# t0saki/YOLO-Infer-pt

Hardware: AMD Instinct MI355X
Metric: images/sec at 640x640 batch32, v11_n (forward + on-device NMS) (higher is better)
Workload: dtype bf16; 1 GPU; yolo_v11_n eval forward + NMS, 640x640, 32 images per GPU per step; per_gpu_batch=32, global_batch=32, image_size=640, parallelism=dp1, nms=on-device, conf 0.001, iou 0.65, max_det 300

## Files before the change

### yolo-infer-pt_amd/csrc/c3k2.hip

```cpp
#include "common.h"
#include "dtypes.h"

namespace yh {

namespace {

typedef float f32x16 __attribute__((ext_vector_type(16)));

template <typename T> struct CMfma;
template <> struct CMfma<__bf16> {
    static __device__ __forceinline__ f32x16 step(const uint4& a, const uint4& b, const f32x16& c) {
        return __builtin_amdgcn_mfma_f32_32x32x16_bf16(__builtin_bit_cast(bf16x8, a), __builtin_bit_cast(bf16x8, b), c, 0,
                                                       0, 0);
    }
};
template <> struct CMfma<_Float16> {
    static __device__ __forceinline__ f32x16 step(const uint4& a, const uint4& b, const f32x16& c) {
        return __builtin_amdgcn_mfma_f32_32x32x16_f16(__builtin_bit_cast(f16x8, a), __builtin_bit_cast(f16x8, b), c, 0, 0,
                                                      0);
    }
};

constexpr int NWV = CSP_THREADS / 64;

__device__ __forceinline__ void cs_glds(const void* src, unsigned lds_addr) {
#if defined(__HIP_DEVICE_COMPILE__)
    unsigned keep;
    asm volatile("s_mov_b32 %0, m0\n\ts_mov_b32 m0, %2\n\ts_nop 0\n\tglobal_load_lds_dwordx4 %1, off\n\ts_mov_b32 m0, %0"
                 : "=&s"(keep) : "v"(src), "s"(lds_addr) : "memory");
#else
    (void)src; (void)lds_addr;
#endif
}
__device__ __forceinline__ void cs_barrier() { asm volatile("s_waitcnt lgkmcnt(0)\n\ts_barrier" ::: "memory"); }

__device__ __forceinline__ uint4 cs_rd(unsigned addr) {
#if defined(__HIP_DEVICE_COMPILE__)
    typedef __attribute__((address_space(3))) const uint4* lp;
    return *reinterpret_cast<lp>((size_t)addr);
#else
    (void)addr;
    return uint4{};
#endif
}
__device__ __forceinline__ void cs_wr(unsigned addr, uint4 v) {
#if defined(__HIP_DEVICE_COMPILE__)
    typedef __attribute__((address_space(3))) uint4* lp;
    *reinterpret_cast<lp>((size_t)addr) = v;
#else
    (void)addr; (void)v;
#endif
}
__device__ __forceinline__ float4 cs_rdf(unsigned addr) {
    const uint4 u = cs_rd(addr);
    return make_float4(__uint_as_float(u.x), __uint_as_float(u.y), __uint_as_float(u.z), __uint_as_float(u.w));
}

struct CsLayout {
    int w1, w2, w3, w4, b1, b2, b3, b4, prm;
};
__host__ __device__ constexpr CsLayout cs_layout(int ni, int nc, int no) {
    const int nh = (nc + 1) / 2, na3 = (nc + 1) / 2;
    CsLayout L{};
    L.w1 = 0;
    L.w2 = L.w1 + nc * ni * 1024;
    L.w3 = L.w2 + 9 * nc * 1024;
    L.w4 = L.w3 + na3 * 9 * nh * 1024;
    L.b1 = L.w4 + no * 3 * nc * 1024;
    L.b2 = L.b1 + 32 * nc * 4;
    L.b3 = L.b2 + 32 * 4;
    L.b4 = L.b3 + 32 * na3 * 4;
    L.prm = (L.b4 + 32 * no * 4 + 1023) & ~1023;
    return L;
}
struct CsTile {
    int lx, lt, lr, lc, total;
};
__host__ __device__ inline CsTile cs_tile(int TH, int TW, int ni, int nc, int no) {
    const int nh = (nc + 1) / 2;
    const CsLayout L = cs_layout(ni, nc, no);
    const int XP = (TH + 4) * (TW + 4), MP = (TH + 2) * (TW + 2), NP = TH * TW;
    CsTile t{};
    t.lx = L.prm;
    t.lt = t.lx + (ni ? ((XP * (16 * ni + 8) * 2 + 1023) & ~1023) : 0);
    t.lr = t.lt + XP * (32 * nc + 8) * 2;
    t.lc = t.lr + MP * (16 * nh + 8) * 2;
    t.total = t.lc + NP * (16 * nc + 8) * 2;
    return t;
}

template <typename T>
__device__ __forceinline__ void cs_act(const f32x16& acc, unsigned bias_addr, uint4 (&o)[2]) {
    float v[16];
#pragma unroll
    for (int q = 0; q < 4; ++q) {
        const float4 b = cs_rdf(bias_addr + 16 * q);
        v[4 * q] = acc[4 * q] + b.x;
        v[4 * q + 1] = acc[4 * q + 1] + b.y;
        v[4 * q + 2] = acc[4 * q + 2] + b.z;
        v[4 * q + 3] = acc[4 * q + 3] + b.w;
    }
    T t[16];
#pragma unroll
    for (int i = 0; i < 16; ++i) t[i] = fromf<T>(silu<T>(v[i]));
    o[0] = *reinterpret_cast<const uint4*>(&t[0]);
    o[1] = *reinterpret_cast<const uint4*>(&t[8]);
}

template <typename T, int NA, int NK, typename BAddr, typename Epi>
__device__ __forceinline__ void cs_phase(unsigned aimg, int npx, BAddr baddr, Epi epi) {
    const int lane = threadIdx.x & 63, wv = threadIdx.x >> 6, l32 = lane & 31;
    const int items = NA * ((npx + 31) >> 5);
    for (int i0 = wv; i0 < items; i0 += 2 * NWV) {
        const int i1 = i0 + NWV;
        const int a0 = i0 % NA, a1 = i1 % NA;
        const int p0 = (i0 / NA) * 32 + l32, p1 = (i1 / NA) * 32 + l32;
        const int c0 = p0 < npx ? p0 : npx - 1, c1 = p1 < npx ? p1 : npx - 1;
        const unsigned ai0 = aimg + (unsigned)(a0 * NK * 1024 + lane * 16);
        const unsigned ai1 = aimg + (unsigned)(a1 * NK * 1024 + lane * 16);
        f32x16 acc0, acc1;
#pragma unroll
        for (int e = 0; e < 16; ++e) { acc0[e] = 0.f; acc1[e] = 0.f; }
        if (i1 < items) {
#pragma unroll
            for (int k = 0; k < NK; ++k) {
                const uint4 f0 = cs_rd(ai0 + k * 1024), f1 = NA > 1 ? cs_rd(ai1 + k * 1024) : f0;
                const uint4 x0 = cs_rd(baddr(c0, k)), x1 = cs_rd(baddr(c1, k));
                acc0 = CMfma<T>::step(f0, x0, acc0);
                acc1 = CMfma<T>::step(f1, x1, acc1);
            }
            if (p0 < npx) epi(a0, p0, acc0);
            if (p1 < npx) epi(a1, p1, acc1);
        } else {
#pragma unroll
            for (int k = 0; k < NK; ++k) acc0 = CMfma<T>::step(cs_rd(ai0 + k * 1024), cs_rd(baddr(c0, k)), acc0);
            if (p0 < npx) epi(a0, p0, acc0);
        }
    }
}

template <typename T, int NI, int NC, int NO>
__global__ __launch_bounds__(CSP_THREADS) void csp_fused(const CspArgs A) {
    constexpr int NH = (NC + 1) / 2, NA3 = (NC + 1) / 2;
    constexpr int SX = 16 * NI + 8, ST = 32 * NC + 8, SR = 16 * NH + 8, SC = 16 * NC + 8;
    constexpr CsLayout L = cs_layout(NI, NC, NO);
    extern __shared__ __attribute__((aligned(16))) char sm[];
    typedef __attribute__((address_space(3))) char* lds_c;
    const unsigned lds0 = (unsigned)(size_t)(lds_c)sm;
    const int TH = A.TH, TW = A.TW, XW = TW + 4, MW = TW + 2;
    const int XP = (TH + 4) * XW, MP = (TH + 2) * MW, NP = TH * TW;
    const CsTile G = cs_tile(TH, TW, NI, NC, NO);
    const unsigned LX = lds0 + G.lx, LT = lds0 + G.lt, LR = lds0 + G.lr, LC = lds0 + G.lc;
    const int lane = threadIdx.x & 63, hh = lane >> 5;
    const int wvu = __builtin_amdgcn_readfirstlane(threadIdx.x >> 6);
    const T* x = reinterpret_cast<const T*>(A.x);
    T* y = reinterpret_cast<T*>(A.y);

    {
        const char* prm = reinterpret_cast<const char*>(A.prm);
        for (int i0 = wvu * 64; i0 < L.prm / 16; i0 += CSP_THREADS) cs_glds(prm + (size_t)(i0 + lane) * 16, lds0 + i0 * 16);
    }
    constexpr bool TAIL = NI == 0;
    constexpr int NCH = TAIL ? 4 * NC : 2 * NI;
    constexpr int CPX = NCH + 1;
    const unsigned LD = TAIL ? LT : LX;
    auto load_x = [&](int t) {
        const int n = t / A.tiles, tix = t - n * A.tiles;
        const int ty = tix / A.ntw, tx = tix - ty * A.ntw;
        const int h0 = ty * TH - 2, w0 = tx * TW - 2;
        const int total = XP * CPX;
        for (int i0 = wvu * 64; i0 < total; i0 += CSP_THREADS) {
            const int q = i0 + lane;
            const int px = q / CPX, c = q - px * CPX;
            const int r = px / XW, cc = px - r * XW;
            const int gh = h0 + r, gw = w0 + cc;
            const bool ok = q < total && c < NCH && (unsigned)gh < (unsigned)A.H && (unsigned)gw < (unsigned)A.W;
            const void* src = ok ? (const void*)(x + (((long long)n * A.H + gh) * A.W + gw) * A.ldx + c * 8) : A.zero;
            cs_glds(src, LD + i0 * 16);
        }
    };
    const int t0 = xcd_remap(blockIdx.x, gridDim.x);
    if (t0 < A.ntiles) load_x(t0);

    for (int t = t0; t < A.ntiles; t += gridDim.x) {
        const int n = t / A.tiles, tix = t - n * A.tiles;
        const int ty = tix / A.ntw, tx = tix - ty * A.ntw;
        const int h0 = ty * TH, w0 = tx * TW;
        asm volatile("s_waitcnt vmcnt(0)" ::: "memory");
        cs_barrier();

        if constexpr (!TAIL) {
        cs_phase<T, NC, NI>(
                lds0 + L.w1, XP,
                [&](int px, int k) { return LX + (unsigned)(px * SX + 16 * k + 8 * hh) * 2; },
                [&](int a, int px, const f32x16& acc) {
                    uint4 o[2];
                    cs_act<T>(acc, lds0 + L.b1 + (32 * a + 16 * hh) * 4, o);
                    const int r = px / XW, cc = px - r * XW;
                    const int gh = h0 - 2 + r, gw = w0 - 2 + cc;
                    if (!((unsigned)gh < (unsigned)A.H && (unsigned)gw < (unsigned)A.W)) o[0] = o[1] = make_uint4(0, 0, 0, 0);
                    const unsigned d = LT + (unsigned)(px * ST + 32 * a + 16 * hh) * 2;
                    cs_wr(d, o[0]);
                    cs_wr(d + 16, o[1]);
                });
        cs_barrier();
        if (t + (int)gridDim.x < A.ntiles) load_x(t + gridDim.x);
        }

        cs_phase<T, 1, 9 * NC>(
            lds0 + L.w2, MP,
            [&](int px, int k) {
                const int cb = k / 9, tap = k - 9 * (k / 9), kh = tap / 3, kw = tap - 3 * (tap / 3);
                const int r = px / MW, cc = px - r * MW;
                return LT + (unsigned)(((r + kh) * XW + cc + kw) * ST + 16 * NC + 16 * cb + 8 * hh) * 2;
            },
            [&](int, int px, const f32x16& acc) {
                if (16 * hh >= 16 * NH) return;
                uint4 o[2];
                cs_act<T>(acc, lds0 + L.b2 + 16 * hh * 4, o);
                const int r = px / MW, cc = px - r * MW;
                const int gh = h0 - 1 + r, gw = w0 - 1 + cc;
                if (!((unsigned)gh < (unsigned)A.H && (unsigned)gw < (unsigned)A.W)) o[0] = o[1] = make_uint4(0, 0, 0, 0);
                const unsigned d = LR + (unsigned)(px * SR + 16 * hh) * 2;
                cs_wr(d, o[0]);
                cs_wr(d + 16, o[1]);
            });
        cs_barrier();

        cs_phase<T, NA3, 9 * NH>(
                lds0 + L.w3, NP,
                [&](int px, int k) {
                    const int cb = k / 9, tap = k - 9 * (k / 9), kh = tap / 3, kw = tap - 3 * (tap / 3);
                    const int r = px / TW, cc = px - r * TW;
                    return LR + (unsigned)(((r + kh) * MW + cc + kw) * SR + 16 * cb + 8 * hh) * 2;
                },
                [&](int a, int px, const f32x16& acc) {
                    const int co = 32 * a + 16 * hh;
                    if (co >= 16 * NC) return;
                    uint4 o[2];
                    cs_act<T>(acc, lds0 + L.b3 + co * 4, o);
                    const int r = px / TW, cc = px - r * TW;
                    const unsigned rs = LT + (unsigned)(((r + 2) * XW + cc + 2) * ST + 16 * NC + co) * 2;
#pragma unroll
                    for (int hf = 0; hf < 2; ++hf) {
                        const uint4 rv = cs_rd(rs + 16 * hf);
                        const T* ov = reinterpret_cast<const T*>(&o[hf]);
                        const T* rr = reinterpret_cast<const T*>(&rv);
                        T s[8];
#pragma unroll
                        for (int e = 0; e < 8; ++e) s[e] = fromf<T>(tof(ov[e]) + tof(rr[e]));
                        o[hf] = *reinterpret_cast<const uint4*>(s);
                    }
                    const unsigned d = LC + (unsigned)(px * SC + co) * 2;
                    cs_wr(d, o[0]);
                    cs_wr(d + 16, o[1]);
                });
        cs_barrier();

        cs_phase<T, NO, 3 * NC>(
                lds0 + L.w4, NP,
                [&](int px, int k) {
                    const int r = px / TW, cc = px - r * TW;
                    return k < 2 * NC ? LT + (unsigned)(((r + 2) * XW + cc + 2) * ST + 16 * k + 8 * hh) * 2
                                      : LC + (unsigned)(px * SC + 16 * (k - 2 * NC) + 8 * hh) * 2;
                },
                [&](int a, int px, const f32x16& acc) {
                    uint4 o[2];
                    const int co = 32 * a + 16 * hh;
                    cs_act<T>(acc, lds0 + L.b4 + co * 4, o);
                    const int r = px / TW, cc = px - r * TW;
                    const int gh = h0 + r, gw = w0 + cc;
                    if ((unsigned)gh < (unsigned)A.H && (unsigned)gw < (unsigned)A.W) {
                        uint4* d = reinterpret_cast<uint4*>(y + (((long long)n * A.H + gh) * A.W + gw) * A.ldy + co);
                        d[0] = o[0];
                        d[1] = o[1];
                    }
                });
        if constexpr (TAIL) {
            cs_barrier();
            if (t + (int)gridDim.x < A.ntiles) load_x(t + gridDim.x);
        }
    }
    asm volatile("s_waitcnt vmcnt(0)" ::: "memory");
}

#define YH_CSP_LIST(X) X(2, 1, 2) X(4, 2, 4) X(0, 2, 2) X(0, 2, 4)

template <typename T>
int launch_csp_t(const CspArgs& a, int grid, hipStream_t s) {
    const int lds = csp_lds(a.TH, a.TW, a.ni, a.nc, a.no);
    if (lds == 0 || grid <= 0 || a.ldx % 8 || a.ldy % 8) return (int)hipErrorInvalidValue;
#define YH_CSP_CASE(NI, NC, NO)                                                                              \
    if (a.ni == NI && a.nc == NC && a.no == NO) {                                                            \
        static bool attr = false;                                                                            \
        if (!attr) {                                                                                         \
            (void)hipFuncSetAttribute(reinterpret_cast<const void*>(&csp_fused<T, NI, NC, NO>),              \
                                      hipFuncAttributeMaxDynamicSharedMemorySize, 160 * 1024);               \
            attr = true;                                                                                     \
        }                                                                                                    \
        hipLaunchKernelGGL((csp_fused<T, NI, NC, NO>), dim3((unsigned)grid), dim3(CSP_THREADS), lds, s, a); \
        return (int)hipGetLastError();                                                                       \
    }
    YH_CSP_LIST(YH_CSP_CASE)
#undef YH_CSP_CASE
    return (int)hipErrorInvalidValue;
}

}

int csp_prm_bytes(int ni, int nc, int no) { return cs_layout(ni, nc, no).prm; }

void csp_offsets(int ni, int nc, int no, int (&off)[9]) {
    const CsLayout L = cs_layout(ni, nc, no);
    const int v[9] = {L.w1, L.w2, L.w3, L.w4, L.b1, L.b2, L.b3, L.b4, L.prm};
    for (int i = 0; i < 9; ++i) off[i] = v[i];
}

int csp_lds(int TH, int TW, int ni, int nc, int no) {
    bool inst = false;
#define YH_CSP_HAS(NI, NC, NO) inst = inst || (ni == NI && nc == NC && no == NO);
    YH_CSP_LIST(YH_CSP_HAS)
#undef YH_CSP_HAS
    if (!inst || TH < 1 || TW < 1) return 0;
    const int b = cs_tile(TH, TW, ni, nc, no).total;
    return b <= 160 * 1024 ? b : 0;
}

int launch_csp(int dtype, const CspArgs& a, int grid, hipStream_t s) {
    switch (dtype) {
        case F16: return launch_csp_t<_Float16>(a, grid, s);
        case BF16: return launch_csp_t<__bf16>(a, grid, s);
    }
    return (int)hipErrorInvalidValue;
}

}
```

### yolo-infer-pt_amd/csrc/engine.cpp

```cpp
#include <hip/hip_runtime.h>

#include <algorithm>
#include <cmath>
#include <cstdio>
#include <cstring>
#include <map>
#include <memory>
#include <stdexcept>
#include <string>
#include <vector>

#include "common.h"
#include "conv_mx.h"
#include "match_host.h"
#include "merge_host.h"
#include "yolo_hip.h"


namespace yh {

static thread_local std::string g_err;

struct Fail : std::runtime_error {
    int code;
// ... 92 lines not shown
    std::vector<Seg> in;
    View out, res;
    bool has_res = false;
    int heads = 0;
    View lvl[3];
    int hc[3][5] = {};
    View hx[3], hy[3];
    bool hlv[3] = {false, false, false};
    bool direct = false;
    int bc[3] = {-1, -1, -1};
    View bx[3];
    int dlo = 0;
    bool dbox = true;
    int cs[4] = {-1, -1, -1, -1};
    int ck[7] = {-1, -1, -1, -1, -1, -1, -1};
    int alt0 = -1, alt1 = -1;
    int bxc[3][3] = {{-1, -1, -1}, {-1, -1, -1}, {-1, -1, -1}};
    std::vector<int> alts;
    struct PwRun { int stage = -1; int coff = 0; int nch = 0; int load = -1; };
    struct PwStage { std::vector<PwRun> runs; int res_stage = -2; int res_coff = 0; int res_load = -1; bool keep = false; int lds = -1; };
    std::vector<PwStage> pws;
    std::vector<View> pwl;
    std::vector<int> pwl_lds;
    int pwP = 0, pwLds = 0;
    std::string label;
};

struct Workspace {
    int B = 0, H = 0, W = 0;
    void* base = nullptr;
    size_t bytes = 0;
    std::vector<size_t> off;
};

struct GraphKey {
    int B, H, W;
    int X = 0;
    bool operator<(const GraphKey& o) const {
        return B != o.B ? B < o.B : (H != o.H ? H < o.H : (W != o.W ? W < o.W : X < o.X));
    }
};

struct Options {
    bool fuse = true, csp_tail = false, tune_log = false, c3k = true, hcls_wide = true, box_chain = false, pw_chain = true;
    int conv_force = -1;
    static Options from_env() {
        Options o;
        if (const char* e = getenv("YH_FUSE")) o.fuse = atoi(e) != 0;
        if (const char* e = getenv("YH_BOXCHAIN")) o.box_chain = atoi(e) != 0;
        if (const char* e = getenv("YH_PWCHAIN")) o.pw_chain = atoi(e) != 0;
        if (const char* e = getenv("YH_CSP_TAIL")) o.csp_tail = atoi(e) != 0;
        if (const char* e = getenv("YH_C3K")) o.c3k = atoi(e) != 0;
        if (const char* e = getenv("YH_HCLS_WIDE")) o.hcls_wide = atoi(e) != 0;
        if (const char* e = getenv("YH_CONV")) o.conv_force = atoi(e);
        o.tune_log = getenv("YH_TUNE_LOG") != nullptr;
        return o;
    }
};

struct Net {
    yh_variant var;
    Options opt;
    int device, dtype, es;
    std::vector<Tensor> tensors;
    std::vector<ConvDesc> convs;
    std::vector<Op> ops;
    Workspace ws;
    void** io_dev = nullptr;
    void* zero_dev = nullptr;
    bool use_graph = true;
    std::map<GraphKey, hipGraphExec_t> graphs;
    hipStream_t cap_stream = nullptr;
    bool profile = false;
    std::vector<double> prof_ms;
    std::vector<int> prof_calls;
    GraphKey prof_key{0, 0, 0};
    std::vector<hipEvent_t> ev;
    int lastB = 0, lastH = 0, lastW = 0;
    struct MxChoice { MxPlan plan; const char* w = nullptr; std::string name; };
    std::map<GraphKey, std::vector<MxChoice>> conv_kern;
    const std::vector<MxChoice>* cur_kern = nullptr;
    int force_kern = -1;
    int num_cus = 0;
    struct Unit { int first, last; bool level; };
    struct Plan {
        std::vector<Unit> units;
        std::vector<char> active;
    };
    std::map<GraphKey, Plan> plans;
    const Plan* cur_plan = nullptr;

    int tensor(int level, int C) {
        tensors.push_back({level, round_up(C, 8)});
        return (int)tensors.size() - 1;
    }
    View full(int t, int C = -1) {
        View v;
        v.t = t;
        v.coff = 0;
        v.C = C < 0 ? tensors[t].C : C;
        return v;
    }
    View slice(int t, int coff, int C) {
        require(coff % 8 == 0 && C % 8 == 0, "concat slice not a multiple of 8 channels");
        View v;
        v.t = t;
        v.coff = coff;
        v.C = C;
        return v;
    }
    int new_conv(const std::string& name, ConvKind kind, int cin, int cout, int k, int s, int g, int has_bias, int act) {
        ConvDesc d;
        d.name = name;
        d.kind = kind;
        d.cin = cin; d.cout = cout; d.k = k; d.stride = s; d.groups = g;
        d.has_bias = has_bias; d.act = act;
        convs.push_back(std::move(d));
        return (int)convs.size() - 1;
    }
    void dense(const std::string& name, const std::vector<Seg>& in, const std::vector<int>& logical, int cout, int k,
               int s, int act, View out, const View* res = nullptr, int has_bias = 0) {
        int cin = 0;
        for (int c : logical) cin += c;
        const int ci = new_conv(name, CK_DENSE, cin, cout, k, s, 1, has_bias, act);
        ConvDesc& d = convs[ci];
        for (size_t i = 0; i < in.size(); ++i) d.segs.push_back({logical[i], in[i].v.C});
        require(in.size() <= 2, "at most two concat segments");
        if (in.size() == 2) require(logical[0] == in[0].v.C && logical[0] % 8 == 0, "segment 0 must be 8-aligned");
        Op op;
        op.kind = OP_CONV;
        op.conv = ci;
        op.in = in;
        op.out = out;
        if (res) { op.res = *res; op.has_res = true; }
        op.label = name;
        ops.push_back(op);
    }
    View conv1(const std::string& name, View x, int xc, int cout, int act, View out, const View* res = nullptr) {
        dense(name, {Seg{x, 0}}, {xc}, cout, 1, 1, act, out, res);
        return out;
    }
    View conv3(const std::string& name, View x, int xc, int cout, int s, int act, View out, const View* res = nullptr) {
        dense(name, {Seg{x, 0}}, {xc}, cout, 3, s, act, out, res);
        return out;
    }

    void residual(const std::string& p, View x, int ch, double e, View out, int level) {
        const int hid = (int)(ch * e);
        const int t = tensor(level, hid);
        conv3(p + ".conv1", x, ch, hid, 1, ACT_SILU, full(t));
        conv3(p + ".conv2", full(t), hid, ch, 1, ACT_SILU, out, &x);
    }
    void cspmodule(const std::string& p, View x, int in_ch, int out_ch, View out, int level) {
        const int h = out_ch / 2;
        const int t = tensor(level, 2 * h);
        View a = slice(t, 0, h), b = slice(t, h, h);
        const int a0 = tensor(level, h), a1 = tensor(level, h);
        const int first = (int)ops.size();
        conv1(p + ".conv1", x, in_ch, h, ACT_SILU, full(a0));
        conv1(p + ".conv2", x, in_ch, h, ACT_SILU, b);
        residual(p + ".res_m.0", full(a0), h, 1.0, full(a1), level);
        residual(p + ".res_m.1", full(a1), h, 1.0, a, level);
        conv1(p + ".conv3", full(t), 2 * h, out_ch, ACT_SILU, out);
        if (dtype != F32 && opt.fuse && opt.c3k && (in_ch == 64 || in_ch == 128) && out_ch == in_ch && x.C == in_ch &&
            x.coff % 8 == 0 && out.coff % 8 == 0) {
            Op op;
// ... 333 lines not shown
                }
            }
        }
        if ((int)ch.pwl.size() > PWC_MAX_LOADS) return false;
        auto layout = [&](int P) {
            int off = 0;
            for (int k = 0; k < n; ++k) {
                Op::PwStage& st = ch.pws[k];
                st.lds = -1;
                if (!st.keep) continue;
                st.lds = off;
                off += (P * (convs[ops[i + k].conv].cout + 8) * 2 + 15) & ~15;
            }
            ch.pwl_lds.assign(ch.pwl.size(), 0);
            for (size_t z = 0; z < ch.pwl.size(); ++z) {
                off = (off + 1023) & ~1023;
                ch.pwl_lds[z] = off;
                off += (P * (ch.pwl[z].C + 8) * 2 + 1023) & ~1023;
            }
            off = (off + 1023) & ~1023;
            return off + 1024;
        };
        int P = 64, lds = layout(64);
        if (lds > 160 * 1024) {
            P = 32;
            lds = layout(32);
        }
        if (lds > 160 * 1024) return false;
        ch.pwP = P;
        ch.pwLds = lds;
        for (int k = 0; k < n; ++k) ch.alts.push_back((int)(i + k));
        ch.label = ops[i].label + " +" + std::to_string(n - 1);
        ch.out = ops[e - 1].out;
        for (auto& o : ops) {
            if (o.alt0 >= (int)e) o.alt0++;
            if (o.alt1 >= (int)e) o.alt1++;
            for (int& k : o.alts)
                if (k >= (int)e) k++;
        }
        ops.insert(ops.begin() + e, ch);
        return true;
    }
    int new_dense_conv(const std::string& name, int cin, int cout, int k, int has_bias, int act) {
        const int ci = new_conv(name, CK_DENSE, cin, cout, k, 1, 1, has_bias, act);
        convs[ci].segs.push_back({cin, round_up(cin, 8)});
        return ci;
    }
    bool fuse_stem(int c0, int c1, int c2) const {
        if (dtype == F32 || !opt.fuse) return false;
        return c0 == 3 && stem2_ok(c1, c2);
    }
    const void* stem2_params(const Op& op, int& bias_off) {
        ConvDesc& d = convs[op.cs[0]];
        const int nt = d.cout / 32, nk = 9 * (d.cin / 16);
        bias_off = nt * nk * 1024;
        auto it = d.mx_w.find("stem2");
        if (it != d.mx_w.end()) return it->second;
        require(d.loaded, "weights of " + d.name + " not loaded", YH_ESTATE);
        std::vector<uint8_t> img((size_t)bias_off + (size_t)d.cout * 4, 0);
        uint16_t* dst = reinterpret_cast<uint16_t*>(img.data());
        for (int a = 0; a < nt; ++a)
            for (int k = 0; k < nk; ++k)
                for (int lane = 0; lane < 64; ++lane)
                    for (int j = 0; j < 8; ++j) {
                        const int R = lane & 31, hh = lane >> 5;
                        const int co = 32 * a + 16 * ((R >> 2) & 1) + (R & 3) + 4 * (R >> 3);
                        const int cb = k / 9, tap = k - cb * 9, ch = 16 * cb + 8 * hh + j;
                        const float v = d.wf[((size_t)co * d.cin + ch) * 9 + tap];
                        dst[((size_t)(a * nk + k) * 64 + lane) * 8 + j] = dtype == BF16 ? f2bf(v) : f2h(v);
                    }
        float* bd = reinterpret_cast<float*>(img.data() + bias_off);
        for (int i = 0; i < d.cout; ++i) bd[i] = d.bf[i];
        void* dev = nullptr;
        HIPCHECK(hipMalloc(&dev, img.size()));
        HIPCHECK(hipMemcpy(dev, img.data(), img.size(), hipMemcpyHostToDevice));
        d.mx_w.emplace("stem2", dev);
        return dev;
    }
    bool fuse_csp(const std::vector<Seg>& in, const std::vector<int>& logical, int c, int out_ch, View out) const {
        if (dtype == F32 || !opt.fuse) return false;
        if (in.size() != 1 || in[0].up || in[0].v.C != logical[0] || logical[0] % 16 || c % 16 || out_ch % 32) return false;
        if (out.coff % 8 || in[0].v.coff % 8) return false;
        int TH, TW;
        return csp_tile(logical[0] / 16, c / 16, out_ch / 32, 1 << 30, 1 << 30, TH, TW);
    }
    bool fuse_csp_tail(int c, int out_ch, View out) const {
        if (dtype == F32 || !opt.fuse) return false;
        if (c % 16 || out_ch % 32 || out.coff % 8) return false;
        int TH, TW;
        return csp_tile(0, c / 16, out_ch / 32, 1 << 30, 1 << 30, TH, TW);
    }
    bool tail_first() const { return opt.csp_tail; }
    static bool csp_tile(int ni, int nc, int no, int H, int W, int& TH, int& TW) {
        if (const char* e = getenv("YH_CSP_TILE")) {
            int th = 0, tw = 0;
            if (sscanf(e, "%dx%d", &th, &tw) == 2 && th > 0 && tw > 0 && th <= H && tw <= W &&
                csp_lds(th, tw, ni, nc, no) > 0) {
                TH = th;
                TW = tw;
                return true;
            }
        }
        static const int cand[][2] = {{8, 32}, {16, 16}, {8, 16}, {8, 8}, {4, 16}, {4, 8}, {2, 8}, {2, 4}};
        const bool wide = CSP_THREADS >= 1024;
        for (int lim : {80 * 1024, 160 * 1024})
            for (auto& c : cand) {
                if (wide && lim == 80 * 1024) break;
                if (!wide && c[0] * c[1] > 128) continue;
                if (c[0] > H || c[1] > W || (lim == 80 * 1024 && c[0] * c[1] < 64)) continue;
                const int b = csp_lds(c[0], c[1], ni, nc, no);
                if (b > 0 && b <= lim) {
                    TH = c[0];
                    TW = c[1];
                    return true;
                }
            }
        return false;
    }
    const void* csp_params(const Op& op) {
        const int k0 = op.cs[0] >= 0 ? 0 : 1;
        ConvDesc& d0 = convs[op.cs[k0]];
        auto it = d0.mx_w.find("csp");
        bool ok = it != d0.mx_w.end();
        for (int k = k0 + 1; k < 4; ++k) ok = ok && convs[op.cs[k]].mx_w.count("csp_dep");
        if (ok) return it->second;
        if (it != d0.mx_w.end()) {
            (void)hipFree(it->second);
            d0.mx_w.erase(it);
        }
        for (int k = k0; k < 4; ++k) require(convs[op.cs[k]].loaded, "weights of " + convs[op.cs[k]].name + " not loaded", YH_ESTATE);
        const ConvDesc &r1 = convs[op.cs[1]], &r2 = convs[op.cs[2]], &c2 = convs[op.cs[3]];
        const int ni = k0 == 0 ? convs[op.cs[0]].cin / 16 : 0, nc = r1.cin / 16, no = c2.cout / 32, nh = (nc + 1) / 2;
        int off[9];
        csp_offsets(ni, nc, no, off);
        std::vector<uint8_t> img((size_t)off[8], 0);
        auto frags = [&](int o, const ConvDesc& d, int ntile, int nk) {
            const int kk2 = d.k * d.k;
            uint16_t* dst = reinterpret_cast<uint16_t*>(img.data() + o);
            for (int a = 0; a < ntile; ++a)
                for (int k = 0; k < nk; ++k)
                    for (int lane = 0; lane < 64; ++lane)
                        for (int j = 0; j < 8; ++j) {
                            const int R = lane & 31, hh = lane >> 5;
                            const int co = 32 * a + 16 * ((R >> 2) & 1) + (R & 3) + 4 * (R >> 3);
                            const int cb = k / kk2, tap = k - cb * kk2, ch = 16 * cb + 8 * hh + j;
                            float v = 0.f;
                            if (co < d.cout && ch < d.cin) v = d.wf[((size_t)co * d.cin + ch) * kk2 + tap];
                            dst[((size_t)(a * nk + k) * 64 + lane) * 8 + j] = dtype == BF16 ? f2bf(v) : f2h(v);
                        }
        };
        if (ni) frags(off[0], convs[op.cs[0]], nc, ni);
        frags(off[1], r1, 1, 9 * nc);
        frags(off[2], r2, nh, 9 * nh);
        frags(off[3], c2, no, 3 * nc);
        auto biases = [&](int o, const ConvDesc& d) {
            float* dst = reinterpret_cast<float*>(img.data() + o);
            for (int i = 0; i < d.cout; ++i) dst[i] = d.bf[i];
        };
        if (ni) biases(off[4], convs[op.cs[0]]);
        biases(off[5], r1);
        biases(off[6], r2);
        biases(off[7], c2);
        void* dev = nullptr;
        HIPCHECK(hipMalloc(&dev, img.size()));
        HIPCHECK(hipMemcpy(dev, img.data(), img.size(), hipMemcpyHostToDevice));
        d0.mx_w.emplace("csp", dev);
        for (int k = k0 + 1; k < 4; ++k) convs[op.cs[k]].mx_w.emplace("csp_dep", nullptr);
        return dev;
    }
    const void* c3k_params(const Op& op) {
        ConvDesc& d0 = convs[op.ck[0]];
        auto it = d0.mx_w.find("c3k");
        bool ok = it != d0.mx_w.end();
        for (int k = 1; k < 7; ++k) ok = ok && convs[op.ck[k]].mx_w.count("c3k_dep");
        if (ok) return it->second;
        if (it != d0.mx_w.end()) {
            (void)hipFree(it->second);
            d0.mx_w.erase(it);
        }
        for (int k = 0; k < 7; ++k) require(convs[op.ck[k]].loaded, "weights of " + convs[op.ck[k]].name + " not loaded", YH_ESTATE);
        const int hh = convs[op.ck[0]].cout, nt3 = hh / 32, nk1 = hh / 8, nk3 = 9 * hh / 16;
        int off[9];
        c3k_offsets(hh, off);
        std::vector<uint8_t> img((size_t)off[8], 0);
        auto frags = [&](int o, const ConvDesc& d, int ntile, int nk, bool rho) {
            const int kk2 = d.k * d.k;
            uint16_t* dst = reinterpret_cast<uint16_t*>(img.data() + o);
            for (int a = 0; a < ntile; ++a)
                for (int k = 0; k < nk; ++k)
                    for (int lane = 0; lane < 64; ++lane)
                        for (int j = 0; j < 8; ++j) {
// ... 698 lines not shown
                a.H = H; a.W = W; a.Ho = H >> 1; a.Wo = W >> 1;
                a.Cout = d.cout_p;
                a.ldo = ldc(op.out);
                a.M = B * a.Ho * a.Wo;
                a.w = (const float*)d.w_dev;
                a.bias = d.b_dev;
                a.out = ptr(op.out);
                a.act = d.act;
                a.in_u8 = in_u8;
                rc = launch_first_conv(dtype, a, B, s);
                break;
            }
            case OP_CONV: {
                if (dtype != F32) {
                    require(cur_kern != nullptr, "conv plans not chosen", YH_ESTATE);
                    rc = launch_mx_op(op, (*cur_kern)[oi].plan, B, H, W, s);
                    break;
                }
                ConvArgs a{};
                int BM, BN;
                conv_args(op, B, H, W, a, BM, BN);
                rc = launch_conv(dtype, CONV_GEMM, BM, BN, a, s);
                break;
            }
            case OP_DW: rc = launch_dwconv(dtype, dw_args(op, B, H, W), s); break;
            case OP_SPPF: rc = launch_sppf(dtype, pool_args(op, B, H, W), s); break;
            case OP_ATTN: rc = launch_attention(dtype, attn_args(op, H, W), B, s); break;
            case OP_HEADCLS: {
                rc = launch_head_cls(dtype, head_cls_args(op, B, H, W), s);
                break;
            }
            case OP_DECODE: {
                DecodeArgs a{};
                for (int l = 0; l < 3; ++l) {
                    const Tensor& t = tensors[op.lvl[l].t];
                    a.lvl[l] = ptr(op.lvl[l]);
                    a.H[l] = H >> t.level; a.W[l] = W >> t.level;
                    a.stride[l] = (float)(1 << t.level);
                    a.ldc = t.C;
                }
                a.nc = var.num_classes;
                a.A = a.H[0] * a.W[0] + a.H[1] * a.W[1] + a.H[2] * a.W[2];
                a.B = B;
                a.io = (const void* const*)io_dev;
                a.a_lo = anchor_off(op.dlo, H, W);
                a.box = op.dbox ? 1 : 0;
                rc = launch_decode(dtype, a, s);
                break;
            }
            case OP_BOXDFL: rc = launch_box_dfl(dtype, box_dfl_args(op, B, H, W), s); break;
            case OP_BOXCHAIN: rc = launch_box_chain(dtype, box_chain_args(op, B, H, W), s); break;
            case OP_PWCHAIN: rc = launch_pw_chain(dtype, pw_chain_args(op, B, H, W), op.pwLds, s); break;
            case OP_STEM2: {
                const ConvDesc& d = convs[op.conv];
                Stem2Args a{};
                a.io = (const void* const*)io_dev;
                a.H = H; a.W = W; a.Hs = H >> 1; a.Ws = W >> 1; a.Ho = H >> 2; a.Wo = W >> 2; a.B = B;
                a.w1 = (const float*)d.w_dev;
                a.b1 = d.b_dev;
                a.c1 = d.cout; a.c1p = d.cout_p; a.c2 = convs[op.cs[0]].cout;
                a.prm = stem2_params(op, a.prm_bias);
                a.out = ptr(op.out);
                a.ldo = ldc(op.out);
                a.in_u8 = in_u8;
                stem2_tiles(a.Ho, a.Wo, a.ntw, a.nth);
                rc = launch_stem2(dtype, a, s);
                break;
            }
            case OP_CSP: {
                CspArgs a{};
                const View& xv = op.in[0].v;
                const int lv = tensors[xv.t].level;
                a.x = ptr(xv);
                a.ldx = ldc(xv);
                a.y = ptr(op.out);
                a.ldy = ldc(op.out);
                a.H = H >> lv;
                a.W = W >> lv;
                a.B = B;
                a.prm = csp_params(op);
                a.ni = op.cs[0] >= 0 ? convs[op.cs[0]].cin / 16 : 0;
                a.nc = convs[op.cs[1]].cin / 16;
                a.no = convs[op.cs[3]].cout / 32;
                require(csp_tile(a.ni, a.nc, a.no, a.H, a.W, a.TH, a.TW), op.label + ": no LDS tile");
                a.ntw = (a.W + a.TW - 1) / a.TW;
                a.tiles = a.ntw * ((a.H + a.TH - 1) / a.TH);
                a.ntiles = B * a.tiles;
                a.zero = zero_dev;
                if (!num_cus) HIPCHECK(hipDeviceGetAttribute(&num_cus, hipDeviceAttributeMultiprocessorCount, device));
                {
                    const int lds = csp_lds(a.TH, a.TW, a.ni, a.nc, a.no);
                    const int per_cu = CSP_THREADS < 1024 && lds > 0 && lds <= 80 * 1024 ? 2 : 1;
                    rc = launch_csp(dtype, a, std::min(a.ntiles, per_cu * num_cus), s);
                }
                break;
            }
            case OP_C3K: {
                C3kArgs a{};
                const View& xv = op.in[0].v;
                const int lv = tensors[xv.t].level;
                a.x = ptr(xv);
                a.ldx = ldc(xv);
                a.y = ptr(op.out);
                a.ldy = ldc(op.out);
                a.H = H >> lv;
                a.W = W >> lv;
                a.B = B;
                a.prm = c3k_params(op);
                a.hh = convs[op.ck[0]].cout;
                rc = launch_c3k(dtype, a, s);
                break;
            }
        }
        if (rc != 0) throw Fail(YH_EHIP, "launch of " + op.label + " failed: " + hipGetErrorString((hipError_t)rc));
    }

    void free_plans() {
        plans.clear();
        cur_plan = nullptr;
    }
    void ensure_plan(int B, int H, int W) {
        const GraphKey key{B, H, W};
        auto it = plans.find(key);
        if (it != plans.end()) { cur_plan = &it->second; return; }
        Plan pl;
        pl.active.assign(ops.size(), 1);
        for (size_t i = 0; i < ops.size(); ++i) {
            if (ops[i].kind != OP_BOXCHAIN) continue;
            bool fits = true;
            for (int l = 0; l < 3; ++l) {
                const int lv = tensors[ops[i].hx[l].t].level;
                int th, tw;
                fits = fits && bx_tile(H >> lv, W >> lv, th, tw);
            }
            if (fits)
                for (int k : ops[i].alts) pl.active[k] = 0;
            else
                pl.active[i] = 0;
        }
        for (size_t i = 0; i < ops.size(); ++i) {
            if (ops[i].kind != OP_PWCHAIN) continue;
            const int lv = tensors[ops[i].out.t].level;
            const long long M = (long long)B * (H >> lv) * (W >> lv);
            const double grid = (double)((M + ops[i].pwP - 1) / ops[i].pwP);
            double wb = 0;
            for (int k : ops[i].alts) wb += (double)convs[ops[k].conv].cout * convs[ops[k].conv].K * es;
            if (wb * grid <= 160e6)
                for (int k : ops[i].alts) pl.active[k] = 0;
            else
                pl.active[i] = 0;
        }
        for (size_t i = 0; i < ops.size(); ++i) {
            if (ops[i].kind != OP_C3K) continue;
            const int lv = tensors[ops[i].out.t].level;
            if (c3k_lds(H >> lv, W >> lv, convs[ops[i].ck[0]].cout) > 0)
                for (int k = ops[i].alt0; k < ops[i].alt1; ++k) pl.active[k] = 0;
            else
                pl.active[i] = 0;
        }
        for (size_t i = 0; i < ops.size(); ++i)
            if (pl.active[i]) pl.units.push_back(Unit{(int)i, (int)i + 1, false});
        cur_plan = &plans.emplace(key, std::move(pl)).first->second;
    }
    void launch_unit(const Unit& u, int B, int H, int W, hipStream_t s) {
        for (int k = u.first; k < u.last; ++k) launch_op(k, B, H, W, s);
    }

    void run_ops(int B, int H, int W, hipStream_t s) {
        if (!cur_plan) {
            for (size_t i = 0; i < ops.size(); ++i) launch_op(i, B, H, W, s);
            return;
        }
// ... 696 lines not shown
        auto it = n.plans.find(yh::GraphKey{batch, height, width});
        yh::require(it != n.plans.end(), "no forward has run at this shape yet", YH_ESTATE);
        const auto& us = it->second.units;
        yh::require(index >= 0 && index < (int)us.size(), "unit index out of range");
        const bool prof_here = n.prof_key.B == batch && n.prof_key.H == height && n.prof_key.W == width;
        if (first_op) *first_op = us[index].first;
        if (num_ops) *num_ops = us[index].last - us[index].first;
        if (is_level) *is_level = us[index].level ? 1 : 0;
        if (ms_total) *ms_total = prof_here && index < (int)n.prof_ms.size() ? n.prof_ms[index] : 0.0;
        if (calls) *calls = prof_here && index < (int)n.prof_calls.size() ? n.prof_calls[index] : 0;
    });
}

int yh_set_graph(yh_handle* h, int enable) {
    return guarded([&] {
        yh::require(h, "null handle");
        h->net.use_graph = enable != 0;
    });
}

int yh_profile_enable(yh_handle* h, int enable) {
    return guarded([&] {
        yh::require(h, "null handle");
        h->net.profile = enable != 0;
    });
}

int yh_profile_reset(yh_handle* h) {
    return guarded([&] {
        yh::require(h, "null handle");
        std::fill(h->net.prof_ms.begin(), h->net.prof_ms.end(), 0.0);
        std::fill(h->net.prof_calls.begin(), h->net.prof_calls.end(), 0);
    });
}

int yh_force_conv_kernel(yh_handle* h, int kernel) {
    return guarded([&] {
        yh::require(h, "null handle");
        yh::require(kernel >= -1, "conv plan index out of range");
        h->net.force_kern = kernel;
        h->net.conv_kern.clear();
        h->net.cur_kern = nullptr;
        h->net.drop_graphs();
    });
}

int yh_debug_op_desc(const yh_handle* h, int index, int batch, int height, int width, char* buf, size_t size) {
    int len = 0;
    const int rc = guarded([&] {
        yh::require(h && index >= 0 && index < (int)h->net.ops.size(), "op index out of range");
        const std::string s = h->net.op_desc(index, batch, height, width);
        yh::require(buf && size > s.size(), "buffer too small");
        std::memcpy(buf, s.c_str(), s.size() + 1);
        len = (int)s.size();
    });
    return rc == YH_OK ? len : rc;
}

int yh_debug_run_ops(yh_handle* h, const void* x, int x_u8, int batch, int height, int width, void* y, int first,
                     int last, void* stream) {
    return guarded([&] {
        yh::require(h && x && y, "null argument");
        h->net.debug_run(x, x_u8, batch, height, width, y, first, last, (hipStream_t)stream);
    });
}

int yh_debug_operand(const yh_handle* h, int index, int slot, void* dst, size_t dst_bytes, void* stream) {
    return guarded([&] {
        yh::require(h && dst, "null argument");
        HIPCHECK(hipSetDevice(h->net.device));
        h->net.debug_operand(index, slot, dst, dst_bytes, (hipStream_t)stream);
    });
}

int yh_op_count(const yh_handle* h) { return h ? (int)h->net.ops.size() : YH_EINVAL; }

int yh_op_kernel(const yh_handle* h, int index, int batch, int height, int width, const char** name) {
    return guarded([&] {
        yh::require(h && index >= 0 && index < (int)h->net.ops.size(), "op index out of range");
        const yh::Net& n = h->net;
        const yh::Op& op = n.ops[index];
        if (op.kind != yh::OP_CONV) {
            if (name) *name = yh::op_kind_name(op.kind);
            return;
        }
        if (n.dtype == yh::F32) {
            if (name) *name = "gemm_f32";
            return;
        }
        auto it = n.conv_kern.find(yh::GraphKey{batch, height, width});
        yh::require(it != n.conv_kern.end(), "no forward has run at this shape yet", YH_ESTATE);
        if (name) *name = it->second[index].name.c_str();
    });
}

int yh_op_info(const yh_handle* h, int index, int batch, int height, int width, const char** label, int* op_class,
               double* bytes, double* flops, double* ms_total, int* calls) {
    return guarded([&] {
        yh::require(h && index >= 0 && index < (int)h->net.ops.size(), "op index out of range");
        const yh::Net& n = h->net;
        const yh::Op& op = n.ops[index];
        if (label) *label = op.label.c_str();
        if (op_class) *op_class = (int)n.op_class(op);
        double b = 0, f = 0;
        n.op_cost(op, batch, height, width, b, f);
        if (bytes) *bytes = b;
        if (flops) *flops = f;
        double ms = 0.0;
        int nc = 0;
        auto it = n.plans.find(yh::GraphKey{batch, height, width});
        const bool prof_here = n.prof_key.B == batch && n.prof_key.H == height && n.prof_key.W == width;
        if (it != n.plans.end() && prof_here) {
            const auto& us = it->second.units;
            for (size_t u = 0; u < us.size() && u < n.prof_ms.size(); ++u)
                if (!us[u].level && us[u].first == index) { ms = n.prof_ms[u]; nc = n.prof_calls[u]; }
        }
        if (ms_total) *ms_total = ms;
        if (calls) *calls = nc;
    });
}

}
```

Measured before the change: 40700 images/s.

## Cost-model CSP tile selection, relax store wait, and half-width epilogues for single-block stages

Replaces the fixed candidate list for the fused C3k2 tile with a cost model that weighs per-tile fixed overhead against MFMA item count and the number of tile waves over CUs. It also replaces the full vmcnt(0) wait at the top of each tile with a partial wait that lets the previous tile's output stores stay in flight. It adds permlane32-swap based half-width epilogues when the hidden or channel block count is one, so both lane halves do useful work instead of idling. Optional trace instrumentation is compiled out by default. The risks are a poorly calibrated cost model picking bad tiles and subtle correctness problems in the partial wait counting.

```diff
diff --git a/yolo-infer-pt_amd/csrc/c3k2.hip b/yolo-infer-pt_amd/csrc/c3k2.hip
--- a/yolo-infer-pt_amd/csrc/c3k2.hip
+++ b/yolo-infer-pt_amd/csrc/c3k2.hip
@@ -33,6 +33,21 @@
 #endif
 }
 __device__ __forceinline__ void cs_barrier() { asm volatile("s_waitcnt lgkmcnt(0)\n\ts_barrier" ::: "memory"); }
+
+__device__ __forceinline__ void cs_wait_vm(int n) {
+    if (n >= 8) asm volatile("s_waitcnt vmcnt(8)" ::: "memory");
+    else if (n >= 4) asm volatile("s_waitcnt vmcnt(4)" ::: "memory");
+    else if (n >= 2) asm volatile("s_waitcnt vmcnt(2)" ::: "memory");
+    else asm volatile("s_waitcnt vmcnt(0)" ::: "memory");
+}
+
+#ifdef YH_CSP_TRACE
+constexpr int CS_TR = 12, CS_TR_TILES = 16, CS_TR_WG = 256, CS_TR_OPS = 4;
+__device__ unsigned long long csp_trace_buf[CS_TR_OPS * CS_TR_WG * CS_TR_TILES * CS_TR];
+#define CS_STAMP(k) do { if (trp) trp[k] = __builtin_amdgcn_s_memtime(); } while (0)
+#else
+#define CS_STAMP(k) do { } while (0)
+#endif
 
 __device__ __forceinline__ uint4 cs_rd(unsigned addr) {
 #if defined(__HIP_DEVICE_COMPILE__)
@@ -107,6 +122,31 @@
     o[1] = *reinterpret_cast<const uint4*>(&t[8]);
 }
 
+template <typename T>
+__device__ __forceinline__ uint4 cs_act_half(const f32x16& acc, unsigned bias_addr, int hh) {
+#if defined(__HIP_DEVICE_COMPILE__)
+    float v[8];
+#pragma unroll
+    for (int e = 0; e < 8; ++e)
+        v[e] = __uint_as_float(
+            __builtin_amdgcn_permlane32_swap(__float_as_uint(acc[e]), __float_as_uint(acc[8 + e]), false, false)[0]);
+    const float4 b0 = cs_rdf(bias_addr + 32 * hh), b1 = cs_rdf(bias_addr + 32 * hh + 16);
+    v[0] += b0.x; v[1] += b0.y; v[2] += b0.z; v[3] += b0.w;
+    v[4] += b1.x; v[5] += b1.y; v[6] += b1.z; v[7] += b1.w;
+    T t[8];
+#pragma unroll
+    for (int i = 0; i < 8; ++i) {
+        float p = silu<T>(v[i]);
+        asm("" : "+v"(p));
+        t[i] = fromf<T>(p);
+    }
+    return *reinterpret_cast<const uint4*>(&t[0]);
+#else
+    (void)acc; (void)bias_addr; (void)hh;
+    return uint4{};
+#endif
+}
+
 template <typename T, int NA, int NK, typename BAddr, typename Epi>
 __device__ __forceinline__ void cs_phase(unsigned aimg, int npx, BAddr baddr, Epi epi) {
     const int lane = threadIdx.x & 63, wv = threadIdx.x >> 6, l32 = lane & 31;
@@ -138,6 +178,10 @@
         }
     }
 }
+
+#ifdef YH_CSP_TRACE
+constexpr int cs_trace_op(int ni, int, int no) { return ni == 2 ? 0 : ni == 4 ? 1 : no == 2 ? 2 : 3; }
+#endif
 
 template <typename T, int NI, int NC, int NO>
 __global__ __launch_bounds__(CSP_THREADS) void csp_fused(const CspArgs A) {
@@ -182,12 +226,30 @@
     const int t0 = xcd_remap(blockIdx.x, gridDim.x);
     if (t0 < A.ntiles) load_x(t0);
 
+    const int p4_items = NO * ((NP + 31) >> 5);
+    const int p4_stores = wvu < p4_items ? 2 * ((p4_items - wvu + NWV - 1) / NWV) : 0;
+    int young = 0;
+#ifdef YH_CSP_TRACE
+    int trk = 0;
+#endif
     for (int t = t0; t < A.ntiles; t += gridDim.x) {
         const int n = t / A.tiles, tix = t - n * A.tiles;
         const int ty = tix / A.ntw, tx = tix - ty * A.ntw;
         const int h0 = ty * TH, w0 = tx * TW;
-        asm volatile("s_waitcnt vmcnt(0)" ::: "memory");
+#ifdef YH_CSP_TRACE
+        unsigned long long* trp = nullptr;
+        if (threadIdx.x == 0 && blockIdx.x < CS_TR_WG && trk < CS_TR_TILES) {
+            trp = csp_trace_buf + ((size_t)(cs_trace_op(NI, NC, NO) * CS_TR_WG + blockIdx.x) * CS_TR_TILES + trk) * CS_TR;
+            trp[10] = __builtin_amdgcn_s_memrealtime();
+            trp[11] = (unsigned long long)TH | (unsigned long long)TW << 16 | (unsigned long long)(t + 1) << 32;
+        }
+        ++trk;
+#endif
+        CS_STAMP(0);
+        cs_wait_vm(young);
+        CS_STAMP(1);
         cs_barrier();
+        CS_STAMP(2);
 
         if constexpr (!TAIL) {
         cs_phase<T, NC, NI>(
@@ -203,7 +265,9 @@
                     cs_wr(d, o[0]);
                     cs_wr(d + 16, o[1]);
                 });
+        CS_STAMP(3);
         cs_barrier();
+        CS_STAMP(4);
         if (t + (int)gridDim.x < A.ntiles) load_x(t + gridDim.x);
         }
 
@@ -215,6 +279,14 @@
                 return LT + (unsigned)(((r + kh) * XW + cc + kw) * ST + 16 * NC + 16 * cb + 8 * hh) * 2;
             },
             [&](int, int px, const f32x16& acc) {
+                if constexpr (NH == 1) {
+                    uint4 o = cs_act_half<T>(acc, lds0 + L.b2, hh);
+                    const int r = px / MW, cc = px - r * MW;
+                    const int gh = h0 - 1 + r, gw = w0 - 1 + cc;
+                    if (!((unsigned)gh < (unsigned)A.H && (unsigned)gw < (unsigned)A.W)) o = make_uint4(0, 0, 0, 0);
+                    cs_wr(LR + (unsigned)(px * SR + 8 * hh) * 2, o);
+                    return;
+                }
                 if (16 * hh >= 16 * NH) return;
                 uint4 o[2];
                 cs_act<T>(acc, lds0 + L.b2 + 16 * hh * 4, o);
@@ -225,7 +297,9 @@
                 cs_wr(d, o[0]);
                 cs_wr(d + 16, o[1]);
             });
+        CS_STAMP(5);
         cs_barrier();
+        CS_STAMP(6);
 
         cs_phase<T, NA3, 9 * NH>(
                 lds0 + L.w3, NP,
@@ -235,6 +309,18 @@
                     return LR + (unsigned)(((r + kh) * MW + cc + kw) * SR + 16 * cb + 8 * hh) * 2;
                 },
                 [&](int a, int px, const f32x16& acc) {
+                    if constexpr (NC == 1) {
+                        const uint4 o = cs_act_half<T>(acc, lds0 + L.b3, hh);
+                        const int r = px / TW, cc = px - r * TW;
+                        const uint4 rv = cs_rd(LT + (unsigned)(((r + 2) * XW + cc + 2) * ST + 16 * NC + 8 * hh) * 2);
+                        const T* ov = reinterpret_cast<const T*>(&o);
+                        const T* rr = reinterpret_cast<const T*>(&rv);
+                        T s[8];
+#pragma unroll
+                        for (int e = 0; e < 8; ++e) s[e] = fromf<T>(tof(ov[e]) + tof(rr[e]));
+                        cs_wr(LC + (unsigned)(px * SC + 8 * hh) * 2, *reinterpret_cast<const uint4*>(s));
+                        return;
+                    }
                     const int co = 32 * a + 16 * hh;
                     if (co >= 16 * NC) return;
                     uint4 o[2];
@@ -255,7 +341,9 @@
                     cs_wr(d, o[0]);
                     cs_wr(d + 16, o[1]);
                 });
+        CS_STAMP(7);
         cs_barrier();
+        CS_STAMP(8);
 
         cs_phase<T, NO, 3 * NC>(
                 lds0 + L.w4, NP,
@@ -276,6 +364,8 @@
                         d[1] = o[1];
                     }
                 });
+        CS_STAMP(9);
+        if constexpr (!TAIL) young = h0 + TH <= A.H && w0 + TW <= A.W ? p4_stores : 0;
         if constexpr (TAIL) {
             cs_barrier();
             if (t + (int)gridDim.x < A.ntiles) load_x(t + gridDim.x);
@@ -326,6 +416,13 @@
     return b <= 160 * 1024 ? b : 0;
 }
 
+#ifdef YH_CSP_TRACE
+extern "C" int yh_debug_csp_trace(unsigned long long* dst, int n) {
+    if (n > CS_TR_OPS * CS_TR_WG * CS_TR_TILES * CS_TR) n = CS_TR_OPS * CS_TR_WG * CS_TR_TILES * CS_TR;
+    return (int)hipMemcpyFromSymbol(dst, HIP_SYMBOL(csp_trace_buf), (size_t)n * 8, 0, hipMemcpyDeviceToHost);
+}
+#endif
+
 int launch_csp(int dtype, const CspArgs& a, int grid, hipStream_t s) {
     switch (dtype) {
         case F16: return launch_csp_t<_Float16>(a, grid, s);
diff --git a/yolo-infer-pt_amd/csrc/engine.cpp b/yolo-infer-pt_amd/csrc/engine.cpp
--- a/yolo-infer-pt_amd/csrc/engine.cpp
+++ b/yolo-infer-pt_amd/csrc/engine.cpp
@@ -198,6 +198,7 @@
     const std::vector<MxChoice>* cur_kern = nullptr;
     int force_kern = -1;
     int num_cus = 0;
+    std::map<std::pair<GraphKey, int>, std::string> csp_plan;
     struct Unit { int first, last; bool level; };
     struct Plan {
         std::vector<Unit> units;
@@ -697,16 +698,20 @@
         if (in.size() != 1 || in[0].up || in[0].v.C != logical[0] || logical[0] % 16 || c % 16 || out_ch % 32) return false;
         if (out.coff % 8 || in[0].v.coff % 8) return false;
         int TH, TW;
-        return csp_tile(logical[0] / 16, c / 16, out_ch / 32, 1 << 30, 1 << 30, TH, TW);
+        return csp_tile(logical[0] / 16, c / 16, out_ch / 32, 1, 1 << 30, 1 << 30, 1, TH, TW);
     }
     bool fuse_csp_tail(int c, int out_ch, View out) const {
         if (dtype == F32 || !opt.fuse) return false;
         if (c % 16 || out_ch % 32 || out.coff % 8) return false;
         int TH, TW;
-        return csp_tile(0, c / 16, out_ch / 32, 1 << 30, 1 << 30, TH, TW);
+        return csp_tile(0, c / 16, out_ch / 32, 1, 1 << 30, 1 << 30, 1, TH, TW);
     }
     bool tail_first() const { return opt.csp_tail; }
-    static bool csp_tile(int ni, int nc, int no, int H, int W, int& TH, int& TW) {
+    static int csp_items(int TH, int TW, int ni, int nc, int no) {
+        const auto nb = [](int px) { return (px + 31) / 32; };
+        return (ni ? nc * nb((TH + 4) * (TW + 4)) : 0) + nb((TH + 2) * (TW + 2)) + ((nc + 1) / 2 + no) * nb(TH * TW);
+    }
+    static bool csp_tile(int ni, int nc, int no, int B, int H, int W, int cus, int& TH, int& TW) {
         if (const char* e = getenv("YH_CSP_TILE")) {
             int th = 0, tw = 0;
             if (sscanf(e, "%dx%d", &th, &tw) == 2 && th > 0 && tw > 0 && th <= H && tw <= W &&
@@ -716,12 +721,30 @@
                 return true;
             }
         }
-        static const int cand[][2] = {{8, 32}, {16, 16}, {8, 16}, {8, 8}, {4, 16}, {4, 8}, {2, 8}, {2, 4}};
-        const bool wide = CSP_THREADS >= 1024;
+        if (CSP_THREADS >= 1024) {
+            constexpr long long CSP_TILE_FIXED = 7400, CSP_TILE_ITEM = 230;
+            long long best = -1;
+            H = std::min(H, 1 << 12);
+            W = std::min(W, 1 << 12);
+            for (int th : {2, 4, 8, 10, 12, 16}) {
+                if (th > H || (th == 2 && H >= 4)) continue;
+                for (int tw = 4; tw <= W; tw += 4) {
+                    if (csp_lds(th, tw, ni, nc, no) <= 0) break;
+                    const long long nt = (long long)B * ((H + th - 1) / th) * ((W + tw - 1) / tw);
+                    const long long cost = ((nt + cus - 1) / cus) * (CSP_TILE_FIXED + CSP_TILE_ITEM * csp_items(th, tw, ni, nc, no));
+                    if (best < 0 || cost < best) {
+                        best = cost;
+                        TH = th;
+                        TW = tw;
+                    }
+                    if (nt <= cus) break;
+                }
+            }
+            return best >= 0;
+        }
+        static const int cand[][2] = {{8, 16}, {8, 8}, {4, 16}, {4, 8}, {2, 8}, {2, 4}};
         for (int lim : {80 * 1024, 160 * 1024})
             for (auto& c : cand) {
-                if (wide && lim == 80 * 1024) break;
-                if (!wide && c[0] * c[1] > 128) continue;
                 if (c[0] > H || c[1] > W || (lim == 80 * 1024 && c[0] * c[1] < 64)) continue;
                 const int b = csp_lds(c[0], c[1], ni, nc, no);
                 if (b > 0 && b <= lim) {
@@ -1586,12 +1609,13 @@
                 a.ni = op.cs[0] >= 0 ? convs[op.cs[0]].cin / 16 : 0;
                 a.nc = convs[op.cs[1]].cin / 16;
                 a.no = convs[op.cs[3]].cout / 32;
-                require(csp_tile(a.ni, a.nc, a.no, a.H, a.W, a.TH, a.TW), op.label + ": no LDS tile");
+                if (!num_cus) HIPCHECK(hipDeviceGetAttribute(&num_cus, hipDeviceAttributeMultiprocessorCount, device));
+                require(csp_tile(a.ni, a.nc, a.no, B, a.H, a.W, num_cus, a.TH, a.TW), op.label + ": no LDS tile");
+                csp_plan[{GraphKey{B, H, W}, (int)oi}] = "c3k2_t" + std::to_string(a.TH) + "x" + std::to_string(a.TW);
                 a.ntw = (a.W + a.TW - 1) / a.TW;
                 a.tiles = a.ntw * ((a.H + a.TH - 1) / a.TH);
                 a.ntiles = B * a.tiles;
                 a.zero = zero_dev;
-                if (!num_cus) HIPCHECK(hipDeviceGetAttribute(&num_cus, hipDeviceAttributeMultiprocessorCount, device));
                 {
                     const int lds = csp_lds(a.TH, a.TW, a.ni, a.nc, a.no);
                     const int per_cu = CSP_THREADS < 1024 && lds > 0 && lds <= 80 * 1024 ? 2 : 1;
@@ -2454,6 +2478,8 @@
         const yh::Op& op = n.ops[index];
         if (op.kind != yh::OP_CONV) {
             if (name) *name = yh::op_kind_name(op.kind);
+            auto cp = n.csp_plan.find({yh::GraphKey{batch, height, width}, index});
+            if (name && cp != n.csp_plan.end()) *name = cp->second.c_str();
             return;
         }
         if (n.dtype == yh::F32) {
```

After: 41410 images/s (median of 6 runs). +1.7%, better.
